# zdebruine/singlet

Hardware: AMD Instinct MI355X
Metric: ALS iterations/sec (1M cells x 30k genes, 5% nnz, k=50) (higher is better)
Workload: dtype f64

## Files before the change

singlet_amd/csrc/gen_nnls_lane.py:

```python
#!/usr/bin/env python3
import os
import sys

KPS = [int(a) for a in sys.argv[1:]] or [50]


def plan(KP):
    NG = (KP + 15) // 16
    NGP = (NG + 1) & ~1
    xa = 20 + 4 + 4 * NG + 4 * KP + 16 > 256
    nt = 26 if xa else 20
    own = nt + 4 + 4 * NG + (2 * KP if xa else 4 * KP)
    acc = 2 * KP if xa else 0
    if 16 + own > 256 or KP > 64:
        raise SystemExit("gen_nnls_lane.py: KP = %d does not fit the register file" % KP)
    waves = lambda vt: max(1, min(8, 512 // ((vt + own + acc + 7) // 8 * 8)))
    V_T = max(range(16, min(28, 256 - own) + 1), key=lambda vt: (min(waves(vt), 3), vt))
    V_D = V_T + nt
    V_G = V_D + 4
    V_B = V_G + 4 * NG
    V_X = V_B + 2 * KP
    TOP = V_X if xa else V_X + 2 * KP
    total = TOP + (2 * KP if xa else 0)
    return dict(KP=KP, NG=NG, NGP=NGP, V_T=V_T, V_D=V_D, V_G=V_G, V_B=V_B, V_X=V_X, TOP=TOP, XA=xa, NT=nt,
                WAVES=max(1, min(8, 512 // ((total + 7) // 8 * 8))))


def r2(b):
    return f"v[{b}:{b + 1}]"


class Sweep:
    def __init__(self, KP):
        p = plan(KP)
        self.__dict__.update(p)
        T = self.V_T
        self.A, self.E2 = T, T + 2
        self.ND = [T + 4, T + 6]
        self.DEN, self.R, self.E, self.Q = T + 8, T + 10, T + 12, T + 14
        self.TOL = T + 16
        self.GM = T + 18
        self.XH = [T + 20, T + 22]
        self.XN = T + 24
        self.L = []

    def b(self, j):
        return self.V_B + 2 * j

    def x(self, j):
        return self.V_X + 2 * j

    def g(self, par, m):
        return self.V_G + 2 * self.NG * par + 2 * m

    def head(self, i):
        A, E2, ND = self.A, self.E2, self.ND[i & 1]
        b, gii, rii = self.b(i), self.V_D, self.V_D + 2
        x = self.XH[i & 1] if self.XA else self.x(i)
        ops = []
        if self.XA:
            ops += [f"v_accvgpr_read_b32 v{x}, a{2 * i}", f"v_accvgpr_read_b32 v{x + 1}, a{2 * i + 1}"]
        ops += [
            f"v_mul_f64 {r2(A)}, {r2(b)}, {r2(rii)}",
            f"v_fma_f64 {r2(E2)}, -{r2(A)}, {r2(gii)}, {r2(b)}",
            f"v_fma_f64 {r2(A)}, {r2(E2)}, {r2(rii)}, {r2(A)}",
        ]
        if i + 1 < self.KP:
            ops.append(f"ds_read_b128 v[{self.V_D}:{self.V_D + 3}], %[dl] offset:{16 * (i + 1)}")
        ops += [
            f"v_add_f64 {r2(A)}, {r2(A)}, -%[l1]",
            f"v_fma_f64 {r2(A)}, %[l2], {r2(x)}, {r2(A)}",
            f"v_mul_f64 {r2(A)}, {r2(A)}, {r2(self.GM)}",
            f"v_min_f64 {r2(ND)}, -{r2(A)}, {r2(x)}",
            f"v_cmp_lt_f64_e64 s[{{c0}}:{{c0p}}], {r2(x)}, -{r2(A)}",
            f"v_cmp_neq_f64_e32 vcc, 0, {r2(x)}",
            "s_and_b64 s[{c0}:{c0p}], vcc, s[{c0}:{c0p}]",
        ]
        return ops

    def tail(self, i):
        ND, DEN, R, E, Q = self.ND[i & 1], self.DEN, self.R, self.E, self.Q
        if self.XA:
            xo, x = self.XH[i & 1], self.XN
            first = [f"v_add_f64 {r2(x)}, {r2(xo)}, -{r2(ND)}", f"v_accvgpr_write_b32 a{2 * i}, v{x}", f"v_accvgpr_write_b32 a{2 * i + 1}, v{x + 1}"]
        else:
            x = self.x(i)
            first = [f"v_add_f64 {r2(x)}, {r2(x)}, -{r2(ND)}"]
        return first + [
            f"v_add_f64 {r2(DEN)}, {r2(x)}, %[eps]",
            f"v_rcp_f64 {r2(R)}, {r2(DEN)}",
            f"v_fma_f64 {r2(E)}, -{r2(DEN)}, {r2(R)}, 1.0",
            f"v_fma_f64 {r2(R)}, {r2(R)}, {r2(E)}, {r2(R)}",
            f"v_fma_f64 {r2(E)}, -{r2(DEN)}, {r2(R)}, 1.0",
            f"v_fma_f64 {r2(R)}, {r2(R)}, {r2(E)}, {r2(R)}",
            f"v_mul_f64 {r2(Q)}, {r2(ND)}, {r2(R)}",
            f"v_fma_f64 {r2(E)}, -{r2(DEN)}, {r2(Q)}, {r2(ND)}",
            f"v_fma_f64 {r2(Q)}, {r2(E)}, {r2(R)}, {r2(Q)}",
            f"v_add_f64 {r2(Q)}, {r2(self.TOL)}, |{r2(Q)}|",
            "TOLSEL",
        ]

    def fma(self, i, j):
        return (f"v_fmac_f64_dpp {r2(self.b(j))}, {r2(self.g(i & 1, j >> 4))}, {r2(self.ND[i & 1])} "
                f"row_newbcast:{j & 15} row_mask:0xf bank_mask:0xf")

    def row_reads(self, i):
        out, base = [], 16 * self.NGP * 8 * i
        m = 0
        while m < self.NG:
            if m + 1 < self.NG:
                out.append(f"ds_read_b128 v[{self.g(i & 1, m)}:{self.g(i & 1, m) + 3}], %[gl] offset:{base + 8 * m}")
                m += 2
            else:
                out.append(f"ds_read_b64 {r2(self.g(i & 1, m))}, %[gl] offset:{base + 8 * m}")
                m += 1
        return out

    def emit(self, s, cmp_slot):
        if s == "TOLSEL":
            c0 = 40 + 2 * (cmp_slot & 1)
            self.L.append(f"v_cndmask_b32_e64 v{self.TOL}, v{self.Q}, 0, s[{c0}:{c0 + 1}]")
            self.L.append(f"v_cndmask_b32_e64 v{self.TOL + 1}, v{self.Q + 1}, %[one_hi], s[{c0}:{c0 + 1}]")
            return
        c0 = 40 + 2 * (cmp_slot & 1)
        if self.L and self.L[-1].startswith("v_rcp_f64") and r2(self.R) in s:
            self.L.append("s_nop 0")
        self.L.append(s.replace("{c0}", str(c0)).replace("{c0p}", str(c0 + 1)))

    def build(self):
        KP = self.KP
        L = self.L
        L.append(f"ds_read_b128 v[{self.V_D}:{self.V_D + 3}], %[dl]")
        L.extend(self.row_reads(0))
        L.append("s_waitcnt lgkmcnt(0)")
        for op in self.head(0):
            self.emit(op, 0)
        for i in range(KP):
            L.append("s_waitcnt lgkmcnt(0)")
            if i + 1 < KP:
                L.extend(self.row_reads(i + 1))
            chain = []
            tl = [(op, i) for op in self.tail(i)]
            hd = [(op, i + 1) for op in self.head(i + 1)] if i + 1 < KP else []
            while tl or hd:
                if hd:
                    chain.append(hd.pop(0))
                if tl:
                    chain.append(tl.pop(0))
            order = ([i + 1] if i + 1 < KP else []) + [j for j in range(KP) if j != i + 1]
            nf = 0
            stride = int(os.environ.get("SGL_GEN_NNLS_STRIDE", "2"))
            for j in order:
                L.append(self.fma(i, j))
                nf += 1
                if nf >= 2 and nf % stride == 0 and chain:
                    op, slot = chain.pop(0)
                    self.emit(op, slot)
            for op, slot in chain:
                self.emit(op, slot)
        return L

    def text(self, L=None):
        return " \\\n".join(f'    "{ins}\\n\\t"' for ins in (L if L is not None else self.L))


def kernel_body(KP):
    s = Sweep(KP)
    s.build()
    sweep = s.L
    L = []
    A = L.append
    go, sv, n0, t0, t1, c1 = "s[46:47]", "s[44:45]", "s48", "s49", "s50", "s[50:51]"
    DEN, R, E, Q, TOL, GM = s.DEN, s.R, s.E, s.Q, s.TOL, s.GM

    def go_mask():
        A(f"v_rcp_f64 {r2(R)}, %[kd]")
        A("s_nop 1")
        A(f"v_fma_f64 {r2(E)}, -%[kd], {r2(R)}, 1.0")
        A(f"v_fma_f64 {r2(R)}, {r2(R)}, {r2(E)}, {r2(R)}")
        A(f"v_fma_f64 {r2(E)}, -%[kd], {r2(R)}, 1.0")
        A(f"v_fma_f64 {r2(R)}, {r2(R)}, {r2(E)}, {r2(R)}")
        A(f"v_mul_f64 {r2(Q)}, {r2(TOL)}, {r2(R)}")
        A(f"v_fma_f64 {r2(E)}, -%[kd], {r2(Q)}, {r2(TOL)}")
        A(f"v_fma_f64 {r2(Q)}, {r2(E)}, {r2(R)}, {r2(Q)}")
        A("v_cmp_gt_u32_e32 vcc, 100, %[it]")
        A("s_nop 3")
        A(f"s_mov_b64 {c1}, vcc")
        A(f"v_cmp_lt_f64_e32 vcc, %[thr], {r2(Q)}")
        A("s_nop 3")
        A(f"s_and_b64 {go}, vcc, {c1}")
        A(f"s_and_b64 {go}, {go}, %[valid]")

    def masked(mask, body, last):
        A(f"s_mov_b64 {sv}, exec")
        A(f"s_and_b64 exec, exec, {mask}")
        L.extend(body)
        A("s_cmp_eq_u32 %[klast], 0")
        A("s_cbranch_scc1 1f")
        A(last)
        A("1:")
        A(f"s_mov_b64 exec, {sv}")

    for r in range(s.V_B, s.TOP):
        A(f"v_mov_b32 v{r}, 0")
    if s.XA:
        for r in range(2 * KP):
            A(f"v_accvgpr_write_b32 a{r}, 0")
    xr = (lambda q: f"a[{2 * q}:{2 * q + 1}]") if s.XA else (lambda q: r2(s.x(q)))
    j = KP - 1
    masked("%[valid]", [f"global_load_dwordx2 {r2(s.b(q))}, %[bp], off offset:{8 * q}" for q in range(KP - 1)],
           f"global_load_dwordx2 {r2(s.b(j))}, %[bp], off offset:{8 * j}")
    masked("%[valid]", [f"global_load_dwordx2 {xr(q)}, %[xp], off offset:{8 * q}" for q in range(KP - 1)],
           f"global_load_dwordx2 {xr(j)}, %[xp], off offset:{8 * j}")
    A("s_waitcnt vmcnt(0)")
    A(f"v_mov_b32 v{TOL}, %[lo]")
    A(f"v_mov_b32 v{TOL + 1}, %[hi]")
    go_mask()
    A(f"s_bcnt1_i32_b64 {n0}, {go}")
    A("2:")
    go_mask()
    A(f"s_cmp_eq_u64 {go}, 0")
    A("s_cbranch_scc1 3f")
    A("s_cmp_eq_u32 %[toend], 1")
    A("s_cbranch_scc1 4f")
    A(f"s_bcnt1_i32_b64 {t0}, {go}")
    A(f"s_lshl_b32 {t0}, {t0}, 3")
    A(f"s_mul_i32 {t1}, {n0}, 3")
    A(f"s_cmp_lt_u32 {t0}, {t1}")
    A("s_cbranch_scc1 3f")
    A("4:")
    A("s_add_u32 %[ran], %[ran], 1")
    A(f"v_cndmask_b32_e64 v{TOL}, v{TOL}, 0, {go}")
    A(f"v_cndmask_b32_e64 v{TOL + 1}, v{TOL + 1}, 0, {go}")
    A(f"v_mov_b32 v{GM}, 0")
    A(f"v_cndmask_b32_e64 v{GM + 1}, 0, %[one_hi], {go}")
    L.extend(sweep)
    A(f"v_cndmask_b32_e64 v{s.A}, 0, 1, {go}")
    A(f"v_add_u32 %[it], %[it], v{s.A}")
    A("s_branch 2b")
    A("3:")
    A(f"v_mov_b32 %[lo], v{TOL}")
    A(f"v_mov_b32 %[hi], v{TOL + 1}")
    masked("%[valid]", [f"global_store_dwordx2 %[xp], {xr(q)}, off offset:{8 * q}" for q in range(KP - 1)],
           f"global_store_dwordx2 %[xp], {xr(j)}, off offset:{8 * j}")
    masked(go, [f"global_store_dwordx2 %[bp], {r2(s.b(q))}, off offset:{8 * q}" for q in range(KP - 1)],
           f"global_store_dwordx2 %[bp], {r2(s.b(j))}, off offset:{8 * j}")
    A(f"s_mov_b64 %[um], {go}")
    A("s_waitcnt vmcnt(0)")
    return s, L


def main():
    out = ["// generated by gen_nnls_lane.py -- do not edit", "#pragma once",
           "#define SGL_NNLS_ASM_INSTANCES(X_) " + " ".join(f"X_({KP})" for KP in KPS)]
    for KP in KPS:
        s, L = kernel_body(KP)
        p = plan(KP)
        out.append(f"// ---- KP = {KP}: T v{p['V_T']}, D v{p['V_D']}, G v{p['V_G']}, B v{p['V_B']}, X v{p['V_X']}")
        out.append(f"#define NNLS_ASM_VT_{KP} {p['V_T']}")
        out.append(f"#define NNLS_ASM_NGP_{KP} {p['NGP']}")
        out.append(f"#define NNLS_ASM_WAVES_{KP} {p['WAVES']}")
        out.append(f"#define NNLS_ASM_VCLOB_{KP} " + ", ".join([f'"v{r}"' for r in range(p['V_T'], p['TOP'])] +
                                                                ([f'"a{r}"' for r in range(2 * KP)] if p['XA'] else [])))
        out.append(f"#define NNLS_ASM_BODY_{KP} \\\n{s.text(L)}")
        out.append("")
    sys.stdout.write("\n".join(out) + "\n")


if __name__ == "__main__":
    main()
```

singlet_amd/csrc/kernels_nnls.hip:

```cpp
#include "sgl_internal.h"
#include "nnls_static_for.h"
#include "nnls_quad_global.h"
#include <algorithm>
#include <cstdlib>
#include <utility>
#include <type_traits>

int k_nnls_lane_launch1(hipStream_t s, const double* Gpad, int KP, double* B, double* X, const int64_t* col_nnz, int k,
                        int64_t ncols, double L1, double L2, unsigned long long* sweep_counter, const NnlsPass& ps, dim3 g,
                        dim3 b);
int k_nnls_lane_launch2(hipStream_t s, const double* Gpad, int KP, double* B, double* X, const int64_t* col_nnz, int k,
                        int64_t ncols, double L1, double L2, unsigned long long* sweep_counter, const NnlsPass& ps, dim3 g,
                        dim3 b);
int k_nnls_half_launch(hipStream_t s, const double* Gpad, int KP, double* B, double* X, const int64_t* col_nnz, int k,
                       int64_t ncols, double L1, double L2, unsigned long long* sweep_counter, const NnlsPass& ps);
bool nnls_half_asm_has(int KP, double L1);
int k_nnls_half_launch_asm(hipStream_t s, const double* Gpad, int KP, double* B, double* X, const int64_t* col_nnz, int k,
                           int64_t ncols, double L1, double L2, unsigned long long* sweep_counter, const NnlsPass& ps);
bool nnls_lane_asm_has(int KP, double L1, int64_t ncols);
int k_nnls_lane_launch_asm(hipStream_t s, const double* Gpad, int KP, double* B, double* X, const int64_t* col_nnz, int k,
                           int64_t ncols, double L1, double L2, unsigned long long* sweep_counter, const NnlsPass& ps, dim3 g, dim3 b);

int64_t nnls_repack_min_cols(bool two_lane) {
    const char* e = getenv("SGL_NNLS_REPACK_MIN_COLS");
    const long long x = e ? atoll(e) : 0;
    return (int64_t)(x > 0 ? x : (two_lane ? (1 << 17) : (1 << 18)));
}

int nnls_gram_stride(int KP) { return KP > 40 ? (KP + 15) / 16 * 16 : KP; }
int nnls_lane_kp(int k, double L1) {
    if (k <= 64) return (k + 1) / 2 * 2;
    if (k > SGL_LANE_NNLS_MAX_K) return 0;
    const int kp4 = (k + 3) / 4 * 4;
    return nnls_half_asm_has(kp4, L1) ? kp4 : (k + 7) / 8 * 8;
}

int nnls_scratch_alloc(NnlsScratch& sc, int64_t cap, int k) {
    nnls_scratch_free(sc);
    if (cap < nnls_repack_min_cols(k > 64)) return SGL_OK;
    if (sgl_pool_malloc(&sc.list[0], sizeof(int32_t) * cap) != hipSuccess || sgl_pool_malloc(&sc.list[1], sizeof(int32_t) * cap) != hipSuccess ||
        sgl_pool_malloc(&sc.counts, sizeof(uint32_t) * (SGL_NNLS_MAX_PASSES + 1)) != hipSuccess ||
        sgl_pool_malloc(&sc.it_state, (size_t)cap) != hipSuccess || sgl_pool_malloc(&sc.tol_state, sizeof(double) * cap) != hipSuccess) {
        (void)hipGetLastError();
        nnls_scratch_free(sc);
        sgl_set_error("NNLS scratch: out of device memory");
        return SGL_ENOMEM;
    }
    sc.cap = cap;
    return SGL_OK;
}

void nnls_scratch_free(NnlsScratch& sc) {
    if (sc.list[0]) (void)sgl_pool_free(sc.list[0]);
    if (sc.list[1]) (void)sgl_pool_free(sc.list[1]);
    if (sc.counts) (void)sgl_pool_free(sc.counts);
    if (sc.it_state) (void)sgl_pool_free(sc.it_state);
    if (sc.tol_state) (void)sgl_pool_free(sc.tol_state);
    if (sc.prev_it) (void)sgl_pool_free(sc.prev_it);
    if (sc.packed) (void)sgl_pool_free(sc.packed);
    if (sc.sort_ws) (void)sgl_pool_free(sc.sort_ws);
    sc = NnlsScratch();
}

#define SGL_PACK_BINS 128
#define SGL_PACK_CPB 2048
__global__ __launch_bounds__(256) void nnls_pack_hist_kernel(const uint8_t* __restrict__ key, int64_t n, int nblocks, uint32_t* __restrict__ hist) {
    __shared__ unsigned h[SGL_PACK_BINS];
    if (threadIdx.x < SGL_PACK_BINS) h[threadIdx.x] = 0;
    __syncthreads();
    const int64_t c0 = (int64_t)blockIdx.x * SGL_PACK_CPB;
    for (int q = threadIdx.x; q < SGL_PACK_CPB; q += 256) {
        const int64_t c = c0 + q;
        if (c < n) atomicAdd(&h[key[c] & (SGL_PACK_BINS - 1)], 1u);
    }
    __syncthreads();
    if (threadIdx.x < SGL_PACK_BINS) hist[(size_t)(SGL_PACK_BINS - 1 - threadIdx.x) * nblocks + blockIdx.x] = h[threadIdx.x];
}
__global__ __launch_bounds__(1024) void nnls_pack_scan_kernel(uint32_t* __restrict__ hist, int total, uint32_t* __restrict__ n_out) {
    __shared__ unsigned part[1024];
    const int per = (total + 1023) / 1024;
    const int a = threadIdx.x * per, b = (a + per < total) ? a + per : total;
    unsigned s = 0;
    {
        int e = a;
        for (; e + 8 <= b; e += 8) {
            unsigned v[8];
#pragma unroll
            for (int q = 0; q < 8; ++q) v[q] = hist[e + q];
#pragma unroll
            for (int q = 0; q < 8; ++q) s += v[q];
        }
        for (; e < b; ++e) s += hist[e];
    }
    part[threadIdx.x] = s;
    __syncthreads();
    for (int off = 1; off < 1024; off <<= 1) {
        const unsigned v = (threadIdx.x >= (unsigned)off) ? part[threadIdx.x - off] : 0u;
        __syncthreads();
        part[threadIdx.x] += v;
        __syncthreads();
    }
    unsigned run = part[threadIdx.x] - s;
    {
        int e = a;
        for (; e + 8 <= b; e += 8) {
            unsigned v[8];
#pragma unroll
            for (int q = 0; q < 8; ++q) v[q] = hist[e + q];
#pragma unroll
            for (int q = 0; q < 8; ++q) { hist[e + q] = run; run += v[q]; }
        }
        for (; e < b; ++e) { const unsigned c = hist[e]; hist[e] = run; run += c; }
    }
    if (threadIdx.x == 1023) *n_out = part[1023];
}
__global__ __launch_bounds__(256) void nnls_pack_scatter_kernel(const uint8_t* __restrict__ key, int64_t n, int nblocks,
                                                                const uint32_t* __restrict__ offs, int32_t* __restrict__ packed) {
    __shared__ unsigned cur[SGL_PACK_BINS];
    if (threadIdx.x < SGL_PACK_BINS) cur[threadIdx.x] = offs[(size_t)(SGL_PACK_BINS - 1 - threadIdx.x) * nblocks + blockIdx.x];
    __syncthreads();
    const int64_t c0 = (int64_t)blockIdx.x * SGL_PACK_CPB;
    for (int q = threadIdx.x; q < SGL_PACK_CPB; q += 256) {
        const int64_t c = c0 + q;
        if (c < n) packed[atomicAdd(&cur[key[c] & (SGL_PACK_BINS - 1)], 1u)] = (int32_t)c;
    }
}

int nnls_pack_alloc(NnlsScratch& sc, int64_t ncols) {
    if (sc.prev_it && sc.pack_cap >= ncols) return SGL_OK;
    if (sc.prev_it) (void)sgl_pool_free(sc.prev_it);
    if (sc.packed) (void)sgl_pool_free(sc.packed);
    if (sc.sort_ws) (void)sgl_pool_free(sc.sort_ws);
    sc.prev_it = nullptr; sc.packed = nullptr; sc.sort_ws = nullptr; sc.pack_cap = 0;
    const int64_t nblocks = (ncols + SGL_PACK_CPB - 1) / SGL_PACK_CPB;
    if (sgl_pool_malloc(&sc.prev_it, (size_t)ncols) != hipSuccess || sgl_pool_malloc(&sc.packed, sizeof(int32_t) * (size_t)ncols) != hipSuccess ||
        sgl_pool_malloc(&sc.sort_ws, sizeof(uint32_t) * ((size_t)SGL_PACK_BINS * nblocks + 4)) != hipSuccess ||
        hipMemset(sc.prev_it, 0, (size_t)ncols) != hipSuccess) {
        (void)hipGetLastError();
        sgl_set_error("NNLS packing scratch: out of device memory");
        return SGL_ENOMEM;
    }
    sc.pack_cap = ncols;
    return SGL_OK;
}

static int nnls_pack_order(hipStream_t s, const NnlsScratch& scr, int64_t ncols, const int32_t** order, const uint32_t** count) {
    const int nblocks = (int)((ncols + SGL_PACK_CPB - 1) / SGL_PACK_CPB);
    uint32_t* n_dev = scr.sort_ws + (size_t)SGL_PACK_BINS * nblocks;
    nnls_pack_hist_kernel<<<dim3((unsigned)nblocks), dim3(256), 0, s>>>(scr.prev_it, ncols, nblocks, scr.sort_ws);
    nnls_pack_scan_kernel<<<dim3(1), dim3(1024), 0, s>>>(scr.sort_ws, SGL_PACK_BINS * nblocks, n_dev);
    nnls_pack_scatter_kernel<<<dim3((unsigned)nblocks), dim3(256), 0, s>>>(scr.prev_it, ncols, nblocks, scr.sort_ws, scr.packed);
    HIPCHK(hipGetLastError());
    *order = scr.packed;
    if (count) *count = n_dev;
    return SGL_OK;
}

int k_nnls_lane(hipStream_t s, const double* Gpad, int KP, double* B, double* X, const int64_t* col_nnz, int k,
                int64_t ncols, double L1, double L2, unsigned long long* sweep_counter, const NnlsScratch* scr, bool pack_by_sweeps) {
    if (ncols <= 0) return SGL_OK;
    const bool two_lane = KP > 64;
    const bool half_asm = two_lane && nnls_half_asm_has(KP, L1);
    auto launch_lane = nnls_lane_asm_has(KP, L1, ncols) ? k_nnls_lane_launch_asm : (KP <= 40) ? k_nnls_lane_launch1 : k_nnls_lane_launch2;
    const dim3 g((unsigned)((ncols + 255) / 256)), b(256);
    auto launch = [&](const NnlsPass& ps) {
        return half_asm ? k_nnls_half_launch_asm(s, Gpad, KP, B, X, col_nnz, k, ncols, L1, L2, sweep_counter, ps)
               : two_lane ? k_nnls_half_launch(s, Gpad, KP, B, X, col_nnz, k, ncols, L1, L2, sweep_counter, ps)
                          : launch_lane(s, Gpad, KP, B, X, col_nnz, k, ncols, L1, L2, sweep_counter, ps, g, b);
    };
    const int64_t repack_min = nnls_repack_min_cols(two_lane);
    const bool repack = scr != nullptr && scr->list[0] != nullptr && scr->cap >= ncols && ncols >= repack_min;
    uint8_t* const prev_it =
        pack_by_sweeps && (!two_lane || half_asm) && scr != nullptr && scr->prev_it != nullptr && scr->pack_cap >= ncols ? scr->prev_it : nullptr;
    const int32_t* list0 = nullptr;
    const uint32_t* count0 = nullptr;
    if (prev_it != nullptr && ncols >= 65536 && !getenv("SGL_NNLS_NO_PACK")) SGLCHK(nnls_pack_order(s, *scr, ncols, &list0, &count0));
    if (!repack) {
        NnlsPass one = {};
        one.list = list0;
        one.count = count0;
        one.fresh = (list0 != nullptr && !getenv("SGL_NNLS_NO_SNAKE")) ? 2 : 1;
        one.prev_it = prev_it;
        SGLCHK(launch(one));
        HIPCHK(hipGetLastError());
        return SGL_OK;
    }
    HIPCHK(hipMemsetAsync(scr->counts, 0, sizeof(uint32_t) * (SGL_NNLS_MAX_PASSES + 1), s));
    for (int p = 0; p < SGL_NNLS_MAX_PASSES; ++p) {
        const bool last = (p == SGL_NNLS_MAX_PASSES - 1);
        NnlsPass ps;
        ps.list = p ? scr->list[(p - 1) & 1] : list0;
        ps.count = p ? scr->counts + p : count0;
        ps.fresh = p ? 0 : 1;
        ps.prev_it = prev_it;
        ps.next_list = last ? nullptr : scr->list[p & 1];
        ps.next_count = last ? nullptr : scr->counts + p + 1;
        ps.it_state = scr->it_state;
        ps.tol_state = scr->tol_state;
        ps.final_below = (int32_t)std::min<int64_t>(64 * 1024, repack_min / 4);
        SGLCHK(launch(ps));
        HIPCHK(hipGetLastError());
    }
    return SGL_OK;
}

__device__ __forceinline__ double rl64(double v, int lane) {
    const unsigned long long u = (unsigned long long)__double_as_longlong(v);
    const unsigned lo = (unsigned)__builtin_amdgcn_readlane((int)(unsigned)(u & 0xffffffffull), lane);
    const unsigned hi = (unsigned)__builtin_amdgcn_readlane((int)(unsigned)(u >> 32), lane);
    return __longlong_as_double((long long)(((unsigned long long)hi << 32) | lo));
}

template <int R>
__global__ __launch_bounds__(256) void nnls_wave_kernel(const double* __restrict__ G, int64_t gstride,
                                                        const double* __restrict__ B, double* __restrict__ X,
                                                        const int64_t* __restrict__ col_nnz, int k, int64_t ncols,
                                                        double L1, double L2, unsigned long long* __restrict__ sweep_counter) {
    const int lane = threadIdx.x & 63;
    const int64_t wave = ((int64_t)blockIdx.x * blockDim.x + threadIdx.x) >> 6;
    const int64_t nwaves = ((int64_t)gridDim.x * blockDim.x) >> 6;
    const double kd = (double)k;
    int total_sweeps = 0;
    for (int64_t col = wave; col < ncols; col += nwaves) {
        if (col_nnz != nullptr && col_nnz[col] == 0) continue;
        const double* Gc = G + col * gstride;
        double b[R], x[R], gd[R], rg[R];
        bool irr = false;
#pragma unroll
        for (int r = 0; r < R; ++r) {
            const int j = lane + 64 * r;
            b[r] = (j < k) ? B[col * k + j] : 0.0;
            x[r] = (j < k) ? X[col * k + j] : 0.0;
            gd[r] = (j < k) ? Gc[(int64_t)j * k + j] : 1.0;
            rg[r] = 1.0 / gd[r];
            irr = irr || !__builtin_isnormal(rg[r]);
        }
        const bool any_irr = __ballot(irr) != 0ull;
        double tol = 1.0;
        int it = 0;
        for (; it < 100 && (tol / kd) > 1e-8; ++it) {
            tol = 0.0;
            for (int i = 0; i < k; ++i) {
                const int ir = i >> 6, il = i & 63;
                double bsel = b[0], xsel = x[0], gsel = gd[0], rsel = rg[0];
#pragma unroll
                for (int r = 1; r < R; ++r) {
                    if (ir == r) { bsel = b[r]; xsel = x[r]; gsel = gd[r]; rsel = rg[r]; }
                }
                const double bi = rl64(bsel, il), xi = rl64(xsel, il), gii = rl64(gsel, il), rii = rl64(rsel, il);
                const double diff0 = sgl_nnls_quotient(bi, gii, rii, any_irr);
                double xn = xi, dpen;
                const double nd = sgl_nnls_nd_strict(diff0, xi, true, L1, L2, dpen);
                if (nd != 0.0) {
                    sgl_nnls_apply(dpen, nd, xn, tol);
#pragma unroll
                    for (int r = 0; r < R; ++r) {
                        const int j = lane + 64 * r;
                        if (j < k) b[r] = fma(Gc[(int64_t)i * k + j], nd, b[r]);
                        if (ir == r && il == lane) x[r] = xn;
                    }
                }
            }
        }
        total_sweeps += it;
#pragma unroll
        for (int r = 0; r < R; ++r) {
            const int j = lane + 64 * r;
            if (j < k) X[col * k + j] = x[r];
        }
    }
    sgl_nnls_book_sweeps<false>(sweep_counter, total_sweeps, total_sweeps);
}

template <int J>
__device__ __forceinline__ void nnls_row_bcast3(double bsrc, double xsrc, double rsrc, double& bi, double& xi, double& ri) {
    const int blo = __double2loint(bsrc), bhi = __double2hiint(bsrc), xlo = __double2loint(xsrc), xhi = __double2hiint(xsrc);
    const int rlo = __double2loint(rsrc), rhi = __double2hiint(rsrc);
    int r0, r1, r2, r3, r4, r5;
    asm("s_nop 1\n\t"
        "v_mov_b32_dpp %0, %6 row_newbcast:%12 row_mask:0xf bank_mask:0xf\n\t"
        "v_mov_b32_dpp %1, %7 row_newbcast:%12 row_mask:0xf bank_mask:0xf\n\t"
        "v_mov_b32_dpp %2, %8 row_newbcast:%12 row_mask:0xf bank_mask:0xf\n\t"
        "v_mov_b32_dpp %3, %9 row_newbcast:%12 row_mask:0xf bank_mask:0xf\n\t"
        "v_mov_b32_dpp %4, %10 row_newbcast:%12 row_mask:0xf bank_mask:0xf\n\t"
        "v_mov_b32_dpp %5, %11 row_newbcast:%12 row_mask:0xf bank_mask:0xf"
        : "=&v"(r0), "=&v"(r1), "=&v"(r2), "=&v"(r3), "=&v"(r4), "=&v"(r5)
// ... 290 lines not shown
```

singlet_amd/csrc/nnls_static_for.h:

```cpp
#pragma once
#include "sgl_internal.h"
#include <utility>
#include <type_traits>

template <typename F, int... Is>
__device__ __forceinline__ void static_for_impl(F&& f, std::integer_sequence<int, Is...>) {
    (f(std::integral_constant<int, Is>{}), ...);
}
template <int N, typename F>
__device__ __forceinline__ void static_for(F&& f) {
    static_for_impl(f, std::make_integer_sequence<int, N>{});
}

template <int LO, int HI, typename F>
int sgl_rank_dispatch(int i, F&& f) {
    if constexpr (LO < HI) {
        if (i > LO) return sgl_rank_dispatch<LO + 1, HI>(i, f);
    }
    return f(std::integral_constant<int, LO>{});
}


__device__ __forceinline__ double sgl_div_normal(double x, double y) {
    double r = __builtin_amdgcn_rcp(y);
// ... 34 lines not shown
__device__ __forceinline__ double sgl_nnls_quotient(double bi, double gii, double rii, bool any_irregular) {
    double diff0 = sgl_nnls_markstein(bi, gii, rii);
    if (any_irregular) {
        const double q = bi / gii;
        diff0 = __builtin_isnormal(rii) ? diff0 : q;
    }
    return diff0;
}

__device__ __forceinline__ double sgl_nnls_step(double diff0, double& xi, double& tol, bool go, double L1, double L2) {
    double diff;
    const double nd = sgl_nnls_nd(diff0, xi, go, L1, L2, diff);
    sgl_nnls_apply(diff, nd, xi, tol);
    return nd;
}

template <bool REDUCE = true, typename T>
__device__ __forceinline__ void sgl_nnls_book_sweeps(unsigned long long* __restrict__ sweep_counter, T s, T ran) {
    if (sweep_counter == nullptr) return;
    if constexpr (REDUCE) {
        for (int off = 32; off > 0; off >>= 1) s += __shfl_down(s, off, 64);
    }
    if ((threadIdx.x & 63) == 0 && (s != 0 || ran != 0)) {
        atomicAdd(sweep_counter, (unsigned long long)s);
        atomicAdd(sweep_counter + 2, (unsigned long long)ran);
    }
}

__device__ __forceinline__ void sgl_nnls_packing_key(uint8_t* prev_it, int64_t col, int it) {
    if (prev_it != nullptr) prev_it[col] = (uint8_t)it;
}

#ifndef SGL_NNLS_REPACK_NUM
#define SGL_NNLS_REPACK_NUM 3
#define SGL_NNLS_REPACK_DEN 8
#endif

__device__ __forceinline__ int64_t sgl_nnls_pass_size(const NnlsPass& ps, int64_t ncols) { return ps.list ? (int64_t)*ps.count : ncols; }

struct SglNnlsPassCol {
    int64_t col;
    bool valid;
    bool resume;
    bool to_end;
};
__device__ __forceinline__ SglNnlsPassCol sgl_nnls_pass_entry(const NnlsPass& ps, int64_t n_in, int64_t pos, const int64_t* __restrict__ col_nnz) {
    SglNnlsPassCol pc;
    const bool in_range = pos < n_in;
    pc.col = in_range ? (ps.list ? (int64_t)ps.list[pos] : pos) : 0;
    pc.resume = ps.list != nullptr && !ps.fresh;
    pc.valid = in_range && (pc.resume || col_nnz == nullptr || col_nnz[pc.col] != 0);
    pc.to_end = (ps.next_list == nullptr) || n_in <= (int64_t)ps.final_below;
    return pc;
}
__device__ __forceinline__ void sgl_nnls_pass_state(const NnlsPass& ps, const SglNnlsPassCol& pc, double& tol, int& it) {
    tol = 1.0;
    it = 0;
    if (pc.valid && pc.resume) {
        tol = ps.tol_state[pc.col];
        it = (int)ps.it_state[pc.col];
    }
}
template <unsigned long long LANES, typename SaveB>
__device__ __forceinline__ void sgl_nnls_pass_exit(const NnlsPass& ps, const SglNnlsPassCol& pc, bool unfinished, bool speaks, double tol, int it,
                                                   int ran, unsigned long long* __restrict__ sweep_counter, SaveB&& save_b) {
    if (unfinished) {
        save_b();
        if (speaks) {
            ps.tol_state[pc.col] = tol;
            ps.it_state[pc.col] = (uint8_t)it;
        }
    }
    if (pc.valid && !unfinished && speaks) sgl_nnls_packing_key(ps.prev_it, pc.col, it);
    const unsigned long long um = __ballot(unfinished) & LANES;
    if (um != 0ull) {
        const int lane = threadIdx.x & 63;
        unsigned base = 0;
        if (lane == 0) base = atomicAdd(ps.next_count, (unsigned)__popcll(um));
        base = (unsigned)__builtin_amdgcn_readfirstlane((int)base);
        if (unfinished && speaks) ps.next_list[base + (unsigned)__popcll(um & ((1ull << lane) - 1ull))] = (int32_t)pc.col;
    }
    sgl_nnls_book_sweeps(sweep_counter, (pc.valid && !unfinished && speaks) ? it : 0, ran);
}
```

singlet_amd/csrc/sgl_internal.h:

```cpp
#pragma once
#include <hip/hip_runtime.h>
#include <stdint.h>
#include <stdio.h>
#include <stdarg.h>
#include <atomic>
#include <functional>
#include <vector>
#include <algorithm>

#include "../../include/singlet_hip.h"

#define SGL_WAVE 64
#define SGL_MAX_K 1024
#define SGL_LANE_NNLS_MAX_K 128

void sgl_set_error(const char* fmt, ...);

hipError_t sgl_pool_malloc_raw(void** p, size_t bytes);
template <typename T_>
inline hipError_t sgl_pool_malloc(T_** p, size_t bytes) { return sgl_pool_malloc_raw(reinterpret_cast<void**>(p), bytes); }
hipError_t sgl_pool_free(void* p);
hipError_t sgl_pool_mem_info(size_t* free_b, size_t* total_b);
void sgl_pool_release(void);
size_t sgl_pool_cached_bytes(void);
// ... 3 lines not shown
        hipError_t e__ = (expr);                                                                       \
        if (e__ != hipSuccess) {                                                                       \
            sgl_set_error("%s failed: %s (%s:%d)", #expr, hipGetErrorString(e__), __FILE__, __LINE__); \
            return SGL_EHIP;                                                                           \
        }                                                                                              \
    } while (0)

#define SGLCHK(expr)              \
    do {                          \
        int r__ = (expr);         \
        if (r__ != SGL_OK) return r__; \
    } while (0)

template <auto* F>
int sgl_allow_dynamic_lds(int bytes) {
    static std::atomic<bool> attr_set[64];
    int dev = 0;
    HIPCHK(hipGetDevice(&dev));
    if (dev < 0 || dev >= 64 || !attr_set[dev]) {
        HIPCHK(hipFuncSetAttribute(reinterpret_cast<const void*>(F), hipFuncAttributeMaxDynamicSharedMemorySize, bytes));
        if (dev >= 0 && dev < 64) attr_set[dev] = true;
    }
    return SGL_OK;
}

struct DevCSC {
    double* x = nullptr;
    int32_t* i = nullptr;
    int64_t* p = nullptr;
    int32_t nrow = 0, ncol = 0;
    int64_t nnz = 0;
    int64_t* seg = nullptr;
    int32_t tile_rows = 0, ntiles = 0;
};

struct DevTiled {
    uint32_t* roff = nullptr;
    double* x = nullptr;
    int64_t* cstart = nullptr;
    uint8_t* cnt = nullptr;
    uint16_t* ahead = nullptr;
    uint16_t* gtab = nullptr;
    size_t cap_gtab = 0;
    double* part = nullptr;
    double* xm = nullptr;
    uint64_t xm_seed = 0, xm_inv = 0;
    int xm_mask_t = -1;
    int64_t* seg = nullptr;
    int32_t* perm = nullptr;
    size_t cap_perm = 0;
    int64_t perm_nnz = -1;
    bool balance = true;
    bool range_fastest = false;
    double top_share = 0.0;
    double top_share4 = 0.0;
    size_t cap_roff = 0, cap_x = 0, cap_cstart = 0, cap_cnt = 0, cap_part = 0, cap_xm = 0, cap_seg = 0, cap_ahead = 0;
    bool built = false;
    int64_t builds = 0;
    int64_t src_nnz = -1;
    int32_t TR = 0, T = 0, CW = 0, k = 0, R = 1, tiles_per_range = 0;
    int32_t NB = 0;
    int64_t tail_wg0 = -1;
    int32_t tail_R = 1;
    int32_t NSL = 2;
    int32_t KS = 0;
    int64_t nwb = 0, E = 0, ncol = 0, nrow = 0;
};

struct PhaseEvent {
    int phase;
    hipEvent_t e0, e1;
};

struct NnlsPass {
    const int32_t* list;
    const uint32_t* count;
    int32_t* next_list;
    uint32_t* next_count;
    uint8_t* it_state;
    double* tol_state;
    int32_t final_below;
    int32_t fresh;
    uint8_t* prev_it;
};
struct NnlsScratch {
    int32_t* list[2] = {nullptr, nullptr};
    uint32_t* counts = nullptr;
    uint8_t* it_state = nullptr;
    double* tol_state = nullptr;
    int64_t cap = 0;
    uint8_t* prev_it = nullptr;
    int32_t* packed = nullptr;
    uint32_t* sort_ws = nullptr;
    int64_t pack_cap = 0;
};

#define SGL_ML_KEEP 3
struct DevMaskList {
    int64_t* ptr = nullptr;
    int32_t* idx = nullptr;
    double* val = nullptr;
    bool val_ok = false, val_refused = false;
    size_t cap_ptr = 0, cap_idx = 0, cap_val = 0;
    int64_t ncol = 0, total = 0;
    int32_t nrow = 0;
    uint64_t seed = 0, inv = 0;
    int mask_t = -1;
    int64_t col_off = 0, row_off = 0;
    bool refused = false;
};

#define SGL_GRAPH_HUB 128
#define SGL_GRAPH_SEG 64
struct DevGraph {
    double* x = nullptr;
    int32_t* i = nullptr;
    int64_t* p = nullptr;
    int64_t nnz = 0;
    int32_t n = 0;
    int32_t* seg_col = nullptr;
    int64_t* seg_q0 = nullptr;
    int32_t* hub_col = nullptr;
    int32_t* hub_seg0 = nullptr;
    double* part = nullptr;
    int32_t nseg = 0, nhub = 0;
    double* buf = nullptr;
    int32_t n_src = 0;
    int32_t E = 0;
    int32_t n_exp = 0;
    int32_t* exp = nullptr;
    double* halo = nullptr;
};

struct DevGroupLink {
    double* table = nullptr;
    int32_t* group = nullptr;
    int rows = 0, groups = 0;
};

struct sgl_ctx {
    int device = 0;
    hipStream_t own_stream = nullptr;
    hipStream_t stream = nullptr;

    DevCSC A, At;
    DevTiled TA, TAt;
    bool use_tiled = false;
    int64_t cell_offset = 0, ncells_total = 0;
    int64_t* col_nnz_A = nullptr;
    int64_t* col_nnz_At = nullptr;
    int64_t* col_nnz_At_global = nullptr;
    bool gene_nnz_global = false;

    int k = 0;
    double *W = nullptr, *Wprev = nullptr, *H = nullptr, *d = nullptr;
    double* B = nullptr;
    double* red = nullptr;
    double* G = nullptr;
    double* Gpad = nullptr;
    NnlsScratch nnls_scr;
    bool solve_empty = false;
    double* Adense = nullptr;
    bool dense_gemm = false;
    void* rocblas = nullptr;
    double* link_h = nullptr;
    double* link_w = nullptr;
    int link_h_rows = 0, link_w_rows = 0;
    DevGroupLink glink_h, glink_w;
    DevGraph graph;
    bool dense_input = false;
    DevMaskList ML[2];
    int64_t ml_builds[2] = {0, 0};
    DevMaskList MLkeep[2][SGL_ML_KEEP];
    double* Gcols = nullptr;
    int64_t gcols_chunk = 0;
    double* Wd = nullptr;
    double* Sbuf = nullptr;
// ... 310 lines not shown
```

Before: 42.28.

## Add bounded-tolerance NNLS lane kernel with single-Newton reciprocal and redo pass

Adds a variant of the generated per-lane NNLS assembly that uses one Newton step for the reciprocal and folds the L1/gradient scaling into a single FMA, so each coordinate update needs fewer f64 instructions. The convergence test is evaluated at both ends of an error band. Columns whose stop decision falls inside the band are marked tainted and queued for a redo launch with the exact kernel, and their X is left unstored. In exchange it adds an extra kernel launch, a redo list allocation and memset, and an atomic append path, and it is enabled only when L2 is zero and the rank keeps x in vector registers.

```diff
diff --git a/singlet_amd/csrc/gen_nnls_lane.py b/singlet_amd/csrc/gen_nnls_lane.py
--- a/singlet_amd/csrc/gen_nnls_lane.py
+++ b/singlet_amd/csrc/gen_nnls_lane.py
@@ -26,14 +26,24 @@
                 WAVES=max(1, min(8, 512 // ((total + 7) // 8 * 8))))
 
 
+EPS_RCP = 2.0 ** -13
+
+
+def band(KP):
+    return 2.0 * (EPS_RCP ** 2 + (KP + 4) * 2.0 ** -52)
+
+
 def r2(b):
     return f"v[{b}:{b + 1}]"
 
 
 class Sweep:
-    def __init__(self, KP):
+    def __init__(self, KP, bounded=False):
         p = plan(KP)
         self.__dict__.update(p)
+        self.bounded = bounded
+        if bounded and self.XA:
+            raise SystemExit("gen_nnls_lane.py: the bounded variant has no accumulator-register plan (KP = %d)" % KP)
         T = self.V_T
         self.A, self.E2 = T, T + 2
         self.ND = [T + 4, T + 6]
@@ -42,6 +52,8 @@
         self.GM = T + 18
         self.XH = [T + 20, T + 22]
         self.XN = T + 24
+        if bounded:
+            self.E, self.L1G = self.DEN, T + 12
         self.L = []
 
     def b(self, j):
@@ -67,10 +79,15 @@
         ]
         if i + 1 < self.KP:
             ops.append(f"ds_read_b128 v[{self.V_D}:{self.V_D + 3}], %[dl] offset:{16 * (i + 1)}")
+        if self.bounded:
+            ops.append(f"v_fma_f64 {r2(A)}, {r2(A)}, {r2(self.GM)}, -{r2(self.L1G)}")
+        else:
+            ops += [
+                f"v_add_f64 {r2(A)}, {r2(A)}, -%[l1]",
+                f"v_fma_f64 {r2(A)}, %[l2], {r2(x)}, {r2(A)}",
+                f"v_mul_f64 {r2(A)}, {r2(A)}, {r2(self.GM)}",
+            ]
         ops += [
-            f"v_add_f64 {r2(A)}, {r2(A)}, -%[l1]",
-            f"v_fma_f64 {r2(A)}, %[l2], {r2(x)}, {r2(A)}",
-            f"v_mul_f64 {r2(A)}, {r2(A)}, {r2(self.GM)}",
             f"v_min_f64 {r2(ND)}, -{r2(A)}, {r2(x)}",
             f"v_cmp_lt_f64_e64 s[{{c0}}:{{c0p}}], {r2(x)}, -{r2(A)}",
             f"v_cmp_neq_f64_e32 vcc, 0, {r2(x)}",
@@ -86,6 +103,16 @@
         else:
             x = self.x(i)
             first = [f"v_add_f64 {r2(x)}, {r2(x)}, -{r2(ND)}"]
+        if self.bounded:
+            return first + [
+                f"v_add_f64 {r2(DEN)}, {r2(x)}, %[eps]",
+                f"v_rcp_f64 {r2(R)}, {r2(DEN)}",
+                f"v_fma_f64 {r2(E)}, -{r2(DEN)}, {r2(R)}, 1.0",
+                f"v_fma_f64 {r2(R)}, {r2(R)}, {r2(E)}, {r2(R)}",
+                f"v_mul_f64 {r2(Q)}, {r2(ND)}, {r2(R)}",
+                f"v_add_f64 {r2(Q)}, {r2(self.TOL)}, |{r2(Q)}|",
+                "TOLSEL",
+            ]
         return first + [
             f"v_add_f64 {r2(DEN)}, {r2(x)}, %[eps]",
             f"v_rcp_f64 {r2(R)}, {r2(DEN)}",
@@ -164,8 +191,8 @@
         return " \\\n".join(f'    "{ins}\\n\\t"' for ins in (L if L is not None else self.L))
 
 
-def kernel_body(KP):
-    s = Sweep(KP)
+def kernel_body(KP, bounded=False):
+    s = Sweep(KP, bounded=bounded)
     s.build()
     sweep = s.L
     L = []
@@ -190,6 +217,34 @@
         A("s_nop 3")
         A(f"s_and_b64 {go}, vcc, {c1}")
         A(f"s_and_b64 {go}, {go}, %[valid]")
+
+    def go_mask_bounded():
+        lo_go, hi_go, S, E = "s[40:41]", "s[42:43]", s.A, s.E
+        A(f"v_rcp_f64 {r2(R)}, %[kd]")
+        A("s_nop 1")
+        A(f"v_fma_f64 {r2(E)}, -%[kd], {r2(R)}, 1.0")
+        A(f"v_fma_f64 {r2(R)}, {r2(R)}, {r2(E)}, {r2(R)}")
+        A(f"v_fma_f64 {r2(E)}, -%[kd], {r2(R)}, 1.0")
+        A(f"v_fma_f64 {r2(R)}, {r2(R)}, {r2(E)}, {r2(R)}")
+        for end, sign in ((lo_go, "-"), (hi_go, "")):
+            A(f"v_fma_f64 {r2(S)}, {sign}{r2(TOL)}, %[dlt], {r2(TOL)}")
+            A(f"v_mul_f64 {r2(Q)}, {r2(S)}, {r2(R)}")
+            A(f"v_fma_f64 {r2(E)}, -%[kd], {r2(Q)}, {r2(S)}")
+            A(f"v_fma_f64 {r2(Q)}, {r2(E)}, {r2(R)}, {r2(Q)}")
+            A(f"v_cmp_lt_f64_e64 {end}, %[thr], {r2(Q)}")
+        A("v_cmp_gt_u32_e32 vcc, 100, %[it]")
+        A("s_nop 3")
+        A(f"s_xor_b64 {c1}, {lo_go}, {hi_go}")
+        A(f"s_and_b64 {c1}, {c1}, vcc")
+        A(f"s_and_b64 {c1}, {c1}, %[valid]")
+        A(f"s_or_b64 %[tn], %[tn], {c1}")
+        A(f"s_and_b64 {go}, {lo_go}, {hi_go}")
+        A(f"s_and_b64 {go}, {go}, vcc")
+        A(f"s_and_b64 {go}, {go}, %[valid]")
+        A(f"s_andn2_b64 {go}, {go}, %[tn]")
+
+    if bounded:
+        go_mask = go_mask_bounded
 
     def masked(mask, body, last):
         A(f"s_mov_b64 {sv}, exec")
@@ -234,6 +289,8 @@
     A(f"v_cndmask_b32_e64 v{TOL + 1}, v{TOL + 1}, 0, {go}")
     A(f"v_mov_b32 v{GM}, 0")
     A(f"v_cndmask_b32_e64 v{GM + 1}, 0, %[one_hi], {go}")
+    if bounded:
+        A(f"v_mul_f64 {r2(s.L1G)}, {r2(GM)}, %[l1]")
     L.extend(sweep)
     A(f"v_cndmask_b32_e64 v{s.A}, 0, 1, {go}")
     A(f"v_add_u32 %[it], %[it], v{s.A}")
@@ -241,7 +298,11 @@
     A("3:")
     A(f"v_mov_b32 %[lo], v{TOL}")
     A(f"v_mov_b32 %[hi], v{TOL + 1}")
-    masked("%[valid]", [f"global_store_dwordx2 %[xp], {xr(q)}, off offset:{8 * q}" for q in range(KP - 1)],
+    xm = "%[valid]"
+    if bounded:
+        xm = c1
+        A(f"s_andn2_b64 {c1}, %[valid], %[tn]")
+    masked(xm, [f"global_store_dwordx2 %[xp], {xr(q)}, off offset:{8 * q}" for q in range(KP - 1)],
            f"global_store_dwordx2 %[xp], {xr(j)}, off offset:{8 * j}")
     masked(go, [f"global_store_dwordx2 %[bp], {r2(s.b(q))}, off offset:{8 * q}" for q in range(KP - 1)],
            f"global_store_dwordx2 %[bp], {r2(s.b(j))}, off offset:{8 * j}")
@@ -253,9 +314,14 @@
 def main():
     out = ["// generated by gen_nnls_lane.py -- do not edit", "#pragma once",
            "#define SGL_NNLS_ASM_INSTANCES(X_) " + " ".join(f"X_({KP})" for KP in KPS)]
+    out.append("// the bounded-tol variant: the ranks whose x lives in the vector registers")
+    out.append("#define SGL_NNLS_ASMB_INSTANCES(X_) " + " ".join(f"X_({KP})" for KP in KPS if not plan(KP)["XA"]))
     for KP in KPS:
         s, L = kernel_body(KP)
         p = plan(KP)
+        if not p["XA"]:
+            sb, Lb = kernel_body(KP, bounded=True)
+            out.append(f"#define NNLS_ASMB_BODY_{KP} \\\n{sb.text(Lb)}")
         out.append(f"// ---- KP = {KP}: T v{p['V_T']}, D v{p['V_D']}, G v{p['V_G']}, B v{p['V_B']}, X v{p['V_X']}")
         out.append(f"#define NNLS_ASM_VT_{KP} {p['V_T']}")
         out.append(f"#define NNLS_ASM_NGP_{KP} {p['NGP']}")
diff --git a/singlet_amd/csrc/kernels_nnls.hip b/singlet_amd/csrc/kernels_nnls.hip
--- a/singlet_amd/csrc/kernels_nnls.hip
+++ b/singlet_amd/csrc/kernels_nnls.hip
@@ -20,6 +20,10 @@
 bool nnls_lane_asm_has(int KP, double L1, int64_t ncols);
 int k_nnls_lane_launch_asm(hipStream_t s, const double* Gpad, int KP, double* B, double* X, const int64_t* col_nnz, int k,
                            int64_t ncols, double L1, double L2, unsigned long long* sweep_counter, const NnlsPass& ps, dim3 g, dim3 b);
+bool nnls_lane_asm_bounded_has(int KP, double L1, double L2, int64_t ncols);
+double nnls_lane_asm_bounded_band(int KP);
+int k_nnls_lane_launch_asm_bounded(hipStream_t s, const double* Gpad, int KP, double* B, double* X, const int64_t* col_nnz, int k,
+                                   int64_t ncols, double L1, double dlt, unsigned long long* sweep_counter, const NnlsPass& ps, dim3 g, dim3 b);
 
 int64_t nnls_repack_min_cols(bool two_lane) {
     const char* e = getenv("SGL_NNLS_REPACK_MIN_COLS");
@@ -37,6 +41,15 @@
 
 int nnls_scratch_alloc(NnlsScratch& sc, int64_t cap, int k) {
     nnls_scratch_free(sc);
+    if (k <= 64 && cap > 0) {
+        if (sgl_pool_malloc(&sc.redo_list, sizeof(int32_t) * cap) != hipSuccess || sgl_pool_malloc(&sc.redo_count, sizeof(uint32_t)) != hipSuccess) {
+            (void)hipGetLastError();
+            nnls_scratch_free(sc);
+            sgl_set_error("NNLS scratch: out of device memory");
+            return SGL_ENOMEM;
+        }
+        sc.redo_cap = cap;
+    }
     if (cap < nnls_repack_min_cols(k > 64)) return SGL_OK;
     if (sgl_pool_malloc(&sc.list[0], sizeof(int32_t) * cap) != hipSuccess || sgl_pool_malloc(&sc.list[1], sizeof(int32_t) * cap) != hipSuccess ||
         sgl_pool_malloc(&sc.counts, sizeof(uint32_t) * (SGL_NNLS_MAX_PASSES + 1)) != hipSuccess ||
@@ -56,6 +69,8 @@
     if (sc.counts) (void)sgl_pool_free(sc.counts);
     if (sc.it_state) (void)sgl_pool_free(sc.it_state);
     if (sc.tol_state) (void)sgl_pool_free(sc.tol_state);
+    if (sc.redo_list) (void)sgl_pool_free(sc.redo_list);
+    if (sc.redo_count) (void)sgl_pool_free(sc.redo_count);
     if (sc.prev_it) (void)sgl_pool_free(sc.prev_it);
     if (sc.packed) (void)sgl_pool_free(sc.packed);
     if (sc.sort_ws) (void)sgl_pool_free(sc.sort_ws);
@@ -163,7 +178,10 @@
     const bool half_asm = two_lane && nnls_half_asm_has(KP, L1);
     auto launch_lane = nnls_lane_asm_has(KP, L1, ncols) ? k_nnls_lane_launch_asm : (KP <= 40) ? k_nnls_lane_launch1 : k_nnls_lane_launch2;
     const dim3 g((unsigned)((ncols + 255) / 256)), b(256);
+    const bool bounded = !two_lane && scr != nullptr && scr->redo_list != nullptr && scr->redo_cap >= ncols && nnls_lane_asm_bounded_has(KP, L1, L2, ncols);
+    const double dlt = bounded ? nnls_lane_asm_bounded_band(KP) : 0.0;
     auto launch = [&](const NnlsPass& ps) {
+        if (bounded && ps.redo_list != nullptr) return k_nnls_lane_launch_asm_bounded(s, Gpad, KP, B, X, col_nnz, k, ncols, L1, dlt, sweep_counter, ps, g, b);
         return half_asm ? k_nnls_half_launch_asm(s, Gpad, KP, B, X, col_nnz, k, ncols, L1, L2, sweep_counter, ps)
                : two_lane ? k_nnls_half_launch(s, Gpad, KP, B, X, col_nnz, k, ncols, L1, L2, sweep_counter, ps)
                           : launch_lane(s, Gpad, KP, B, X, col_nnz, k, ncols, L1, L2, sweep_counter, ps, g, b);
@@ -175,20 +193,42 @@
     const int32_t* list0 = nullptr;
     const uint32_t* count0 = nullptr;
     if (prev_it != nullptr && ncols >= 65536 && !getenv("SGL_NNLS_NO_PACK")) SGLCHK(nnls_pack_order(s, *scr, ncols, &list0, &count0));
+    if (bounded) HIPCHK(hipMemsetAsync(scr->redo_count, 0, sizeof(uint32_t), s));
+    auto redo = [&](bool resume) {
+        if (!bounded) return (int)SGL_OK;
+        NnlsPass rd = {};
+        rd.list = scr->redo_list;
+        rd.count = scr->redo_count;
+        rd.fresh = resume ? 0 : 1;
+        rd.prev_it = prev_it;
+        rd.it_state = scr->it_state;
+        rd.tol_state = scr->tol_state;
+        SGLCHK(launch(rd));
+        HIPCHK(hipGetLastError());
+        if (getenv("SGL_NNLS_TRACE_REDO")) {
+            uint32_t n = 0;
+            HIPCHK(hipMemcpyAsync(&n, scr->redo_count, sizeof(n), hipMemcpyDeviceToHost, s));
+            HIPCHK(hipStreamSynchronize(s));
+            fprintf(stderr, "nnls redo: %u of %lld columns (k = %d, band %.3g)\n", n, (long long)ncols, k, dlt);
+        }
+        return (int)SGL_OK;
+    };
     if (!repack) {
         NnlsPass one = {};
         one.list = list0;
         one.count = count0;
         one.fresh = (list0 != nullptr && !getenv("SGL_NNLS_NO_SNAKE")) ? 2 : 1;
         one.prev_it = prev_it;
+        if (bounded) { one.redo_list = scr->redo_list; one.redo_count = scr->redo_count; }
         SGLCHK(launch(one));
         HIPCHK(hipGetLastError());
-        return SGL_OK;
+        return redo(false);
     }
     HIPCHK(hipMemsetAsync(scr->counts, 0, sizeof(uint32_t) * (SGL_NNLS_MAX_PASSES + 1), s));
     for (int p = 0; p < SGL_NNLS_MAX_PASSES; ++p) {
         const bool last = (p == SGL_NNLS_MAX_PASSES - 1);
-        NnlsPass ps;
+        NnlsPass ps = {};
+        if (bounded) { ps.redo_list = scr->redo_list; ps.redo_count = scr->redo_count; }
         ps.list = p ? scr->list[(p - 1) & 1] : list0;
         ps.count = p ? scr->counts + p : count0;
         ps.fresh = p ? 0 : 1;
@@ -201,7 +241,7 @@
         SGLCHK(launch(ps));
         HIPCHK(hipGetLastError());
     }
-    return SGL_OK;
+    return redo(true);
 }
 
 __device__ __forceinline__ double rl64(double v, int lane) {
diff --git a/singlet_amd/csrc/kernels_nnls_asm_bounded.hip b/singlet_amd/csrc/kernels_nnls_asm_bounded.hip
--- /dev/null
+++ b/singlet_amd/csrc/kernels_nnls_asm_bounded.hip
@@ -0,0 +1,96 @@
+#include "sgl_internal.h"
+#include "nnls_static_for.h"
+#include "nnls_lane_gen.inc"
+
+#define SGL_DEFINE_NNLS_ASMB_KERNEL(KP)                                                                                             \
+    __global__ __launch_bounds__(256) __attribute__((amdgpu_waves_per_eu(NNLS_ASM_WAVES_##KP, NNLS_ASM_WAVES_##KP))) void nnls_lane_asmb_kernel_##KP(           \
+        const double* __restrict__ Gpad, int gs_in, double* __restrict__ B, double* __restrict__ X,                                \
+        const int64_t* __restrict__ col_nnz, int k, int64_t ncols, double L1, double dlt,                                          \
+        unsigned long long* __restrict__ sweep_counter, NnlsPass ps) {                                                             \
+        constexpr int NG = (KP + 15) / 16, NGP = NNLS_ASM_NGP_##KP, ROW = 16 * NGP;                                                \
+        const int64_t n_in = sgl_nnls_pass_size(ps, ncols);                                                                         \
+                                                                    \
+        unsigned bx = blockIdx.x;                                                                                                   \
+        if (ps.fresh == 2 && gridDim.x > 256u && gridDim.x <= 512u) {                                                               \
+            const unsigned alone = 512u - gridDim.x;                                                                                \
+            bx = bx >= 256u ? gridDim.x - 1u - (bx - 256u) : (bx < 256u - alone ? alone + bx : bx - (256u - alone));               \
+        }                                                                                                                           \
+        if ((int64_t)bx * blockDim.x >= n_in) return;                                                                               \
+        extern __shared__ __attribute__((aligned(16))) double nnls_asmb_lds[];                                                      \
+        double* const Gl = nnls_asmb_lds;                                                         \
+        double* const Dl = nnls_asmb_lds + KP * ROW;                                                          \
+        for (int e = threadIdx.x; e < KP * ROW; e += blockDim.x) {                                                                  \
+            const int i = e / ROW, r = e - i * ROW, l = r / NGP, m = r - l * NGP, j = l + 16 * m;                                   \
+            Gl[e] = (m < NG && j < KP) ? Gpad[j + gs_in * i] : 0.0;                                                                 \
+        }                                                                                                                           \
+        for (int j = threadIdx.x; j < KP; j += blockDim.x) {                                                                        \
+            Dl[2 * j] = Gpad[j * gs_in + j];                                                                                        \
+            Dl[2 * j + 1] = Gpad[KP * gs_in + j];                                                                                   \
+        }                                                                                                                           \
+        __syncthreads();                                                                                                            \
+        const SglNnlsPassCol pc = sgl_nnls_pass_entry(ps, n_in, (int64_t)bx * blockDim.x + threadIdx.x, col_nnz);                   \
+        double* const bp = B + pc.col * k;                                                                                          \
+        double* const xp = X + pc.col * k;                                                                                          \
+        typedef __attribute__((address_space(3))) char lds_char;                                                                    \
+        const unsigned gl = (unsigned)(uintptr_t)(lds_char*)Gl + (unsigned)(threadIdx.x & 15) * (NGP * 8);                          \
+        const unsigned dl = (unsigned)(uintptr_t)(lds_char*)Dl;                                                                     \
+        const double kd = (double)k;                                                                                                \
+        double tol;                                                                                                                 \
+        int it;                                                                                                                     \
+        sgl_nnls_pass_state(ps, pc, tol, it);                                                                                       \
+        int ran = 0, tlo = __double2loint(tol), thi = __double2hiint(tol);                                                          \
+        unsigned long long um = 0ull, tn = 0ull;                                                                                    \
+        const unsigned long long vm = __ballot(pc.valid);                                                                           \
+        const double eps = 1e-15, thr = 1e-8;                                                                                       \
+        const unsigned one_hi = 0x3ff00000u;                                                                                        \
+        const int toend_s = __builtin_amdgcn_readfirstlane(pc.to_end ? 1 : 0), klast_s = __builtin_amdgcn_readfirstlane(k == KP ? 1 : 0); \
+        asm volatile(NNLS_ASMB_BODY_##KP                                                                                            \
+                     : [it] "+v"(it), [lo] "+v"(tlo), [hi] "+v"(thi), [ran] "+s"(ran), [um] "=&s"(um), [tn] "+s"(tn)                \
+                     : [bp] "v"(bp), [xp] "v"(xp), [gl] "v"(gl), [dl] "v"(dl), [one_hi] "v"(one_hi), [valid] "s"(vm),               \
+                       [l1] "s"(L1), [dlt] "s"(dlt), [eps] "s"(eps), [kd] "s"(kd), [thr] "s"(thr), [toend] "s"(toend_s),           \
+                       [klast] "s"(klast_s)                                                                                         \
+                     : NNLS_ASM_VCLOB_##KP, "s40", "s41", "s42", "s43", "s44", "s45", "s46", "s47", "s48", "s49", "s50", "s51",     \
+                       "vcc", "scc", "memory");                                                                                     \
+        tol = __hiloint2double(thi, tlo);                                                                                           \
+        const bool unfinished = ((um >> (threadIdx.x & 63)) & 1ull) != 0ull;                        \
+        const bool tainted = ((tn >> (threadIdx.x & 63)) & 1ull) != 0ull;                                                           \
+        SglNnlsPassCol pq = pc;                                    \
+        pq.valid = pc.valid && !tainted;                                                                                            \
+        sgl_nnls_pass_exit<~0ull>(ps, pq, unfinished, true, tol, it, ran, sweep_counter, [] {});                                    \
+        sgl_nnls_pass_redo(ps, pc, tainted);                                                                                        \
+    }
+
+SGL_NNLS_ASMB_INSTANCES(SGL_DEFINE_NNLS_ASMB_KERNEL)
+
+bool nnls_lane_asm_has(int KP, double L1, int64_t ncols);
+
+bool nnls_lane_asm_bounded_has(int KP, double L1, double L2, int64_t ncols) {
+    if (L2 != 0.0 || getenv("SGL_NNLS_EXACT_TOL") || !nnls_lane_asm_has(KP, L1, ncols)) return false;
+#define SGL_NNLS_ASMB_HAS(K_) if (KP == K_) return true;
+    SGL_NNLS_ASMB_INSTANCES(SGL_NNLS_ASMB_HAS)
+#undef SGL_NNLS_ASMB_HAS
+    return false;
+}
+
+double nnls_lane_asm_bounded_band(int KP) {
+    const double d0 = 2.0 * (0x1p-26 + (double)(KP + 4) * 0x1p-52);
+    const char* e = getenv("SGL_NNLS_TOL_BAND");
+    const double d = e ? atof(e) : 0.0;
+    return d > d0 ? d : d0;
+}
+
+int k_nnls_lane_launch_asm_bounded(hipStream_t s, const double* Gpad, int KP, double* B, double* X, const int64_t* col_nnz, int k,
+                                   int64_t ncols, double L1, double dlt, unsigned long long* sweep_counter, const NnlsPass& ps, dim3 g, dim3 b) {
+    const int gs_in = nnls_gram_stride(KP);
+#define SGL_NNLS_ASMB_CASE(K_)                                                                                                      \
+    if (KP == K_) {                                                                                                                 \
+        const size_t lds = sizeof(double) * ((size_t)K_ * 16 * NNLS_ASM_NGP_##K_ + 2 * K_);                                         \
+        nnls_lane_asmb_kernel_##K_<<<g, b, lds, s>>>(Gpad, gs_in, B, X, col_nnz, k, ncols, L1, dlt, sweep_counter, ps);             \
+        HIPCHK(hipGetLastError());                                                                                                  \
+        return SGL_OK;                                                                                                              \
+    }
+    SGL_NNLS_ASMB_INSTANCES(SGL_NNLS_ASMB_CASE)
+#undef SGL_NNLS_ASMB_CASE
+    sgl_set_error("k_nnls_lane_asm_bounded: no instance for KP=%d", KP);
+    return SGL_EINVAL;
+}
diff --git a/singlet_amd/csrc/nnls_static_for.h b/singlet_amd/csrc/nnls_static_for.h
--- a/singlet_amd/csrc/nnls_static_for.h
+++ b/singlet_amd/csrc/nnls_static_for.h
@@ -140,3 +140,18 @@
     }
     sgl_nnls_book_sweeps(sweep_counter, (pc.valid && !unfinished && speaks) ? it : 0, ran);
 }
+__device__ __forceinline__ void sgl_nnls_pass_redo(const NnlsPass& ps, const SglNnlsPassCol& pc, bool tainted) {
+    const unsigned long long tm = __ballot(tainted);
+    if (tm == 0ull) return;
+    const int lane = threadIdx.x & 63;
+    unsigned base = 0;
+    if (lane == 0) base = atomicAdd(ps.redo_count, (unsigned)__popcll(tm));
+    base = (unsigned)__builtin_amdgcn_readfirstlane((int)base);
+    if (tainted) {
+        ps.redo_list[base + (unsigned)__popcll(tm & ((1ull << lane) - 1ull))] = (int32_t)pc.col;
+        if (!pc.resume && ps.tol_state != nullptr) {
+            ps.tol_state[pc.col] = 1.0;
+            ps.it_state[pc.col] = 0;
+        }
+    }
+}
diff --git a/singlet_amd/csrc/sgl_internal.h b/singlet_amd/csrc/sgl_internal.h
--- a/singlet_amd/csrc/sgl_internal.h
+++ b/singlet_amd/csrc/sgl_internal.h
@@ -109,6 +109,8 @@
     int32_t final_below;
     int32_t fresh;
     uint8_t* prev_it;
+    int32_t* redo_list;
+    uint32_t* redo_count;
 };
 struct NnlsScratch {
     int32_t* list[2] = {nullptr, nullptr};
@@ -120,6 +122,9 @@
     int32_t* packed = nullptr;
     uint32_t* sort_ws = nullptr;
     int64_t pack_cap = 0;
+    int32_t* redo_list = nullptr;
+    uint32_t* redo_count = nullptr;
+    int64_t redo_cap = 0;
 };
 
 #define SGL_ML_KEEP 3
```

Measured after the change: 42.85 (median of 6 runs). 1.01x the previous value.
